# ivanalberico/End-To-End-Self-Supervised-SLAM

Hardware: AMD Instinct MI355X
Metric: online refinement steps/sec @640x480, seq_len=60 (higher is better)
Workload: dtype f32

## Files before the change

### end-to-end-self-supervised-slam_amd/e2ehip/_lib.py

```python
import ctypes
import os

import torch

_HERE = os.path.dirname(os.path.abspath(__file__))
LIB_PATH = os.path.join(os.path.dirname(_HERE), "lib", "libe2eslam_hip.so")

c_fp = ctypes.c_void_p
c_int = ctypes.c_int
c_i64 = ctypes.c_int64
c_f32 = ctypes.c_float


class Strides(ctypes.Structure):
    _fields_ = [("sb", c_i64), ("sc", c_i64), ("sh", c_i64), ("sw", c_i64)]


class WgradReduceDesc(ctypes.Structure):
    _fields_ = [("slabs", c_fp), ("dw", c_fp), ("dbias", c_fp), ("scale", c_fp)] + \
               [(n, c_int) for n in ("S", "Mpad", "Npad", "Cout", "Cin", "KH", "KW", "has_bias", "accumulate", "zl")] + [("first_item", ctypes.c_longlong)]


class CopyDesc(ctypes.Structure):
    _fields_ = [("src", c_fp), ("dst", c_fp), ("bytes", ctypes.c_longlong), ("first_item", ctypes.c_longlong)]


class E2EError(RuntimeError):
    pass


SIGNATURES = {
    "e2e_version": [],
    "e2e_last_error": [],
    "e2e_backproject_fwd": [c_fp, c_fp, c_fp, c_int, c_int, c_int, c_fp],
    "e2e_backproject_bwd": [c_fp, c_fp, c_fp, c_int, c_int, c_int, c_fp],
    "e2e_project3d_fwd": [c_fp, c_fp, c_fp, c_fp, c_fp, c_fp, c_int, c_int, c_int, c_fp],
    "e2e_project3d_bwd": [c_fp, c_fp, c_fp, c_fp, c_fp, c_fp, c_int, c_int, c_int, c_fp],
    "e2e_grid_sample_fwd": [c_fp, Strides, c_fp, c_fp] + [c_int] * 8 + [c_fp],
    "e2e_grid_sample_bwd": [c_fp, Strides, c_fp, c_fp, c_fp, c_fp] + [c_int] * 8 + [c_fp],
    "e2e_grid_sample_bwd_exact": [c_fp, Strides, c_fp, c_fp, c_fp, c_fp, c_fp] + [c_int] * 8 + [c_fp],
    "e2e_photometric_fwd": [c_fp, Strides, c_fp, Strides, c_fp, c_fp, c_int, c_int, c_int, c_int, c_fp],
    "e2e_photometric_bwd": [c_fp, Strides, c_fp, Strides, c_fp, c_fp, c_fp, c_int, c_int, c_int, c_int, c_fp],
    "e2e_warp_photo_workspace_floats": [c_int, c_int, c_int],
    "e2e_warp_photo_fwd": [c_fp, c_fp, Strides, c_fp, Strides, c_fp, c_fp, c_fp, c_fp, c_fp, c_fp, c_int, c_int, c_int,
                           c_fp, c_fp, c_fp, c_fp, c_fp, c_int, c_int, c_int, c_fp],
    "e2e_warp_photo_bwd": [c_fp, c_fp, Strides, c_fp, Strides, c_fp, c_fp, c_fp, c_fp, c_fp, c_int, c_int, c_int,
                           c_fp, c_fp, c_fp, c_fp, c_fp, c_fp, c_int, c_int, c_int, c_fp],
# ... 83 lines not shown
    "e2e_conv2d_bwd_pair_deferred": [c_fp, c_fp, c_int, c_fp] + [c_int] * 13 + [c_fp, c_int, c_fp, c_fp, c_fp, c_fp, c_fp, c_int, c_int, c_fp, c_fp, c_fp,
                                     c_int, c_f32, c_f32, ctypes.POINTER(WgradReduceDesc), c_int, c_fp],
    "e2e_wgrad_reduce_batch_prepare": [ctypes.POINTER(WgradReduceDesc), c_int],
    "e2e_wgrad_reduce_batched": [c_fp, c_int, ctypes.c_longlong, c_fp],
    "e2e_copy_batch_prepare": [ctypes.POINTER(CopyDesc), c_int],
    "e2e_copy_batched": [c_fp, c_int, ctypes.c_longlong, c_fp],
    "e2e_head_bwd_act": [c_fp, c_fp, c_fp, c_fp, c_fp, c_fp, c_fp, c_int, c_int, c_int, c_int, c_int, c_fp],
    "e2e_conv2d_act_bwd_acc": [c_fp, c_fp, c_fp, c_fp, c_i64, c_int, c_int, c_int, c_fp],
    "e2e_conv2d_gather_adjoint": [c_fp] + [c_int] * 7 + [c_fp, c_fp, c_int, c_int, c_fp],
    "e2e_conv2d_wgrad_workspace_floats": [c_int] * 8,
    "e2e_conv2d_bwd_weight": [c_fp, c_fp, c_fp, c_int, c_int, c_fp, c_fp, c_fp] + [c_int] * 13 + [c_f32, c_f32, c_fp],
    "e2e_maxpool3x3s2_fwd": [c_fp, c_fp, c_int, c_int, c_int, c_int, c_fp],
    "e2e_maxpool3x3s2_bwd": [c_fp, c_fp, c_fp, c_int, c_int, c_int, c_int, c_int, c_int, c_fp],
    "e2e_maxpool3x3s2_fwd_idx": [c_fp, c_fp, c_fp, c_int, c_int, c_int, c_int, c_fp],
    "e2e_maxpool3x3s2_bwd_idx": [c_fp, c_fp, c_fp, c_fp, c_int, c_int, c_int, c_int, c_int, c_int, c_fp],
    "e2e_bn_fold": [c_fp, c_fp, c_fp, c_fp, c_f32, c_fp, c_fp, c_fp, c_int, c_fp],
    "e2e_affine_fwd": [c_fp, c_fp, c_fp, c_fp, c_int, c_fp, c_i64, c_int, c_fp],
    "e2e_affine_bwd_workspace_floats": [c_int],
    "e2e_affine_bwd": [c_fp, c_fp, c_fp, c_fp, c_i64, c_int, c_fp, c_fp, c_int, c_fp, c_fp],
    "e2e_upsample2_concat": [c_fp, c_fp, c_fp, c_int, c_int, c_int, c_int, c_int, c_fp],
    "e2e_head_fwd": [c_fp, c_fp, c_fp, c_fp, c_int, c_int, c_int, c_int, c_int, c_fp],
    "e2e_head_workspace_floats": [],
    "e2e_head_bwd": [c_fp, c_fp, c_fp, c_fp, c_fp, c_fp, c_fp, c_int, c_int, c_int, c_int, c_fp],
    "e2e_icp_workspace_bytes": [],
    "e2e_icp_state_doubles": [],
    "e2e_icp_state_init": [c_fp, c_fp, c_fp, c_fp, c_fp, ctypes.c_double, c_fp],
    "e2e_icp_update": [c_fp, c_fp, c_fp, c_fp, c_fp, c_fp, c_int, c_int, ctypes.c_double, ctypes.c_double, ctypes.c_double, ctypes.c_double, c_fp],
    "e2e_icp_reduce_update": [c_fp, c_fp, c_fp, c_fp, c_fp, c_f32, c_i64, c_fp, c_fp, c_fp, c_fp, c_fp, c_fp, c_int, c_int,
                              ctypes.c_double, ctypes.c_double, ctypes.c_double, ctypes.c_double, c_fp],
    "e2e_icp_source_subsample": [c_fp, c_fp, c_int, c_int, c_int, c_fp, c_fp, c_fp],
    "e2e_pf_active_subsample_dev": [c_fp, c_fp, c_fp, c_i64, c_fp, c_int, c_int, c_int, c_fp, c_fp, c_fp, c_i64, c_fp],
    "e2e_icp_normal_equations": [c_fp, c_fp, c_fp, c_fp, c_fp, c_f32, c_i64, c_fp, c_fp, c_fp],
}
_RESTYPE = {"e2e_last_error": ctypes.c_char_p, "e2e_warp_photo_workspace_floats": c_i64,
            "e2e_warp_photo_lossgrad_workspace_floats": c_i64, "e2e_pf_workspace_bytes": c_i64,
            "e2e_warp_photo_terms_lossgrad_workspace_floats": c_i64, "e2e_smoothness_norm_lossgrad_workspace_floats": c_i64,
            "e2e_knn1_workspace_bytes": c_i64, "e2e_knn1_index_capacity_bytes": c_i64, "e2e_knn1_index_capacity_bytes_res": c_i64, "e2e_median_workspace_bytes": c_i64,
            "e2e_depth_scale_workspace_bytes": c_i64, "e2e_reduce_workspace_floats": c_i64,
            "e2e_conv2d_wgrad_workspace_floats": c_i64, "e2e_conv2d_wgrad_tuned_workspace_floats": c_i64, "e2e_conv_tuned_workspace_floats": c_i64, "e2e_conv2d_splitk_workspace_floats": c_i64, "e2e_conv2d_bwd_data_workspace_floats": c_i64,
            "e2e_head_workspace_floats": c_i64, "e2e_icp_workspace_bytes": c_i64, "e2e_icp_state_doubles": c_i64, "e2e_aux_workspace_floats": c_i64,
            "e2e_affine_bwd_workspace_floats": c_i64, "e2e_wgrad_reduce_batch_prepare": ctypes.c_longlong, "e2e_copy_batch_prepare": ctypes.c_longlong}

_lib = None


def load():
    global _lib
    if _lib is None:
        if not os.path.exists(LIB_PATH):
            raise E2EError(f"{LIB_PATH} not found: build it with `python __graft_entry__.py build` "
                           "(there is no CPU / PyTorch fallback for the hot path)")
        lib = ctypes.CDLL(LIB_PATH)
        for name, args in SIGNATURES.items():
            fn = getattr(lib, name)
            fn.argtypes = args
            fn.restype = _RESTYPE.get(name, c_int)
        _lib = lib
    return _lib


PROFILE_HOOK = [None]


def call(name, *args):
    lib = load()
    hook = PROFILE_HOOK[0]
    rc = getattr(lib, name)(*args) if hook is None else hook.around(name, args, lambda: getattr(lib, name)(*args))
    if rc != 0:
        raise E2EError(f"{name} failed ({rc}): {lib.e2e_last_error().decode()}")


def stream():
    return torch.cuda.current_stream().cuda_stream


def dev(t, name="tensor", dtype=torch.float32):
    if not torch.is_tensor(t):
        raise TypeError(f"{name}: expected a torch.Tensor, got {type(t).__name__}")
    if not t.is_cuda:
        raise E2EError(f"{name}: the e2eslam hot path runs on the HIP device only (got a {t.device} tensor); "
                       "there is no CPU fallback")
    if t.dtype != dtype:
        raise TypeError(f"{name}: expected {dtype}, got {t.dtype}")
    return t


def ptr(t):
    return None if t is None else ctypes.c_void_p(t.data_ptr())


def strides4(t):
    s = t.stride()
    return Strides(s[0], s[1], s[2], s[3])
```

### end-to-end-self-supervised-slam_amd/e2ehip/netplan.py

```python
import ctypes
import os

import torch

from . import _lib as L
from .conv import ACT, _ld, epoch_sum

_f32 = torch.float32
PAIR_WGRAD_FIRST = 0


class Buf:
    __slots__ = ("t", "g", "written", "B", "h", "w", "C", "act")

    def __init__(self, B, h, w, C, dev, need_grad=True, act=0):
        self.B, self.h, self.w, self.C = B, h, w, C
        self.act = act
        self.t = torch.empty(B, h, w, C, device=dev, dtype=_f32)
        self.g = torch.empty(B, h, w, C, device=dev, dtype=_f32) if need_grad else None
        self.written = False

    def nchw(self):
        return self.t.permute(0, 3, 1, 2)

# ... 101 lines not shown
        s, s1 = self, self.src1
        L.call("e2e_conv2d_gather_adjoint_act", L.ptr(s.dxp), s.src0.B, s.Hs, s.Ws, s.Cin, s.C1, s.up, 1 if s.pp else 0, L.ptr(s.src0.g),
               L.ptr(s1.g) if s1 is not None else None, 1 if s.src0.written else 0, 1 if (s1 is not None and s1.written) else 0,
               L.ptr(s.src0.t), s.src0.act, L.ptr(s1.t) if s1 is not None else None, s1.act if s1 is not None else 0, st)
        s.src0.written = True
        if s1 is not None:
            s1.written = True


class _Head:

    def __init__(self, plan, src, weight, bias, act):
        self.src, self.weight, self.bias, self.act = src, weight, bias, ACT[act]
        self.out = Buf(src.B, src.h, src.w, 1, plan.dev)
        self.dz = torch.empty_like(self.out.t)
        self.ws = torch.empty(L.load().e2e_head_workspace_floats(), device=plan.dev, dtype=_f32)

    def fwd(self, plan, st, slot=None):
        s = self.src
        L.call("e2e_head_fwd", _at(s.t, slot), L.ptr(self.weight), L.ptr(self.bias), _at(self.out.t, slot), s.B if slot is None else 1, s.h, s.w, s.C, self.act, st)

    def bwd(self, plan, st):
        s, n = self.src, self.out.t.numel()
        L.call("e2e_conv2d_act_bwd", L.ptr(self.out.g), L.ptr(self.out.t), None, L.ptr(self.dz), n, 1, self.act, st)
        if s.written:
            raise RuntimeError("the disparity head's input has a single consumer")
        L.call("e2e_head_bwd_act", L.ptr(self.dz), L.ptr(s.t), L.ptr(self.weight), L.ptr(s.g), L.ptr(plan.sink(self.weight)),
               L.ptr(plan.sink(self.bias)) if self.bias is not None else None, L.ptr(self.ws), s.B, s.h, s.w, s.C, s.act, st)
        s.written = True


class _MaxPool:
    def __init__(self, plan, src):
        self.src = src
        self.out = Buf(src.B, (src.h - 1) // 2 + 1, (src.w - 1) // 2 + 1, src.C, plan.dev)
        self.argmax = torch.empty(self.out.t.shape, device=plan.dev, dtype=torch.uint8)

    def fwd(self, plan, st, slot=None):
        s = self.src
        L.call("e2e_maxpool3x3s2_fwd_idx", _at(s.t, slot), _at(self.out.t, slot), _at(self.argmax, slot), s.B if slot is None else 1, s.h, s.w, s.C, st)

    def bwd(self, plan, st):
        s = self.src
        if s.act not in (0, ACT["relu"]):
            raise NotImplementedError("launch plan: the max-pool follows a ReLU (ResNet stem)")
        L.call("e2e_maxpool3x3s2_bwd_idx", L.ptr(s.t), L.ptr(self.argmax), L.ptr(self.out.g), L.ptr(s.g), s.B, s.h, s.w, s.C, 1 if s.written else 0,
               1 if s.act else 0, st)
        s.written = True


class _BNAffine:

    def __init__(self, plan, src, bn_mod):
        self.src, self.bn = src, bn_mod
        C = src.C
        self.out = Buf(src.B, src.h, src.w, C, plan.dev)
        self.scale, self.shift, self.rstd = (torch.empty(C, device=plan.dev, dtype=_f32) for _ in range(3))
        self.ws = torch.empty(L.load().e2e_affine_bwd_workspace_floats(C), device=plan.dev, dtype=_f32)

    def fwd(self, plan, st, slot=None):
        b, s = self.bn, self.src
        L.call("e2e_bn_fold", L.ptr(b.weight), L.ptr(b.bias), L.ptr(b.running_mean), L.ptr(b.running_var), float(b.eps), L.ptr(self.scale),
               L.ptr(self.shift), L.ptr(self.rstd), s.C, st)
        L.call("e2e_affine_fwd", _at(s.t, slot), L.ptr(self.scale), L.ptr(self.shift), None, 0, _at(self.out.t, slot),
               s.t.numel() if slot is None else s.t[0].numel(), s.C, st)

    def bwd(self, plan, st):
        b, s = self.bn, self.src
        n = s.t.numel()
        L.call("e2e_affine_bwd", L.ptr(self.out.g), L.ptr(s.t), L.ptr(b.running_mean), L.ptr(self.rstd), n // s.C, s.C, L.ptr(plan.sink(b.weight)),
               L.ptr(plan.sink(b.bias)), 0, L.ptr(self.ws), st)
        if s.act != 0:
            raise NotImplementedError("launch plan: a trainable BatchNorm follows a plain convolution")
        L.call("e2e_conv2d_act_bwd_acc", L.ptr(self.out.g), L.ptr(self.out.g), L.ptr(self.scale), L.ptr(s.g), n, s.C, 0, 1 if s.written else 0, st)
        s.written = True


class NetPlan:
    def __init__(self, model, B, H, W, device, overlap=True):
        from depth_estimation.networks import BasicBlock
        self.model, self.dev, self.overlap = model, torch.device(device), overlap
        self.paired = os.environ.get("E2E_PAIRED_BWD", "1") != "0"
        self.B, self.H, self.W = B, H, W
        if H % 32 or W % 32:
            raise ValueError(f"launch plan: the encoder halves the image five times and the decoder doubles it back before every skip "
                             f"concatenation (networks.py:277-292): height and width must be multiples of 32, got {H} x {W}")
        self.ops, self._sinks, self._side = [], {}, None
        enc, dec = model.encoder.encoder, model.decoder
        if any(m.training for m in model.modules() if isinstance(m, torch.nn.BatchNorm2d)):
            raise NotImplementedError("the launch plan runs BatchNorm in eval mode (refinement mode, online_adaption.py:175-184)")
        self.x = Buf(B, H, W, 3, self.dev, need_grad=False)

        def bn_args(bn):
            return (bn.weight, bn.bias, bn.running_mean, bn.running_var, bn.eps)

        def conv_bn(src, conv, bn, relu, residual=None, in_norm=None):
            if bn.weight.requires_grad or bn.bias.requires_grad:
                if relu or residual is not None or in_norm is not None:
                    raise NotImplementedError("launch plan: a trainable BatchNorm is expected on the downsample branches only (set_refinement_mode)")
                z = self._add(_Conv(self, src, None, conv.weight, None, None, None, None, conv.stride[0], conv.padding[0], "zeros", 1, None))
                return self._add(_BNAffine(self, z, bn))
            return self._add(_Conv(self, src, None, conv.weight, None, bn_args(bn), residual, "relu" if relu else None, conv.stride[0],
                                   conv.padding[0], "zeros", 1, in_norm))

        f = conv_bn(self.x, enc.conv1, enc.bn1, True, in_norm=(0.45, 1.0 / 0.225))
# ... 16 lines not shown
                        c2.res_via, c1.pre_from = c1, c2
                elif isinstance(idt_op, _BNAffine) and idt.act == 0:
                    idt.g = c2.out.g
                    c2.res_aliased = True
            feats.append(x)
        self.features = feats
        x = feats[-1]
        for i in range(4, -1, -1):
            c0, c1 = dec.convs[("upconv", i, 0)].conv, dec.convs[("upconv", i, 1)].conv
            x = self._add(_Conv(self, x, None, c0.conv.weight, c0.conv.bias, None, None, "elu", 1, 1, c0.pad_mode, 1, None))
            skip = feats[i - 1] if (dec.use_skips and i > 0) else None
            x = self._add(_Conv(self, x, skip, c1.conv.weight, c1.conv.bias, None, None, "elu", 1, 1, c1.pad_mode, 2, None))
        hc = dec.convs[("dispconv", 0)]
        if tuple(hc.conv.weight.shape) != (1, 16, 3, 3) or hc.pad_mode != "reflect":
            raise NotImplementedError("launch plan: the indoor decoder's 16 -> 1 reflect head")
        self.head = _Head(self, x, hc.conv.weight, hc.conv.bias, "disp")
        self.ops.append(self.head)
        self.disp = self.head.out
        self._desc = None
        self._desc_key = None
        self._retired_tables = []
        self._move_tables = {}
        self._reduce_tables = {}

    def _add(self, op):
        self.ops.append(op)
        return op.out

    def parameters(self):
        out = []
        for op in self.ops:
            if isinstance(op, _Conv) or isinstance(op, _Head):
                out.append(op.weight)
                if op.bias is not None:
                    out.append(op.bias)
            elif isinstance(op, _BNAffine):
                out += [op.bn.weight, op.bn.bias]
        return out

    def sink(self, p):
        s = self._sinks.get(id(p))
        if s is None or s.data_ptr() != _sink_of(p).data_ptr():
            s = self._sinks[id(p)] = _sink_of(p)
            if not s.is_contiguous() or tuple(s.shape) != tuple(p.shape):
                raise RuntimeError("gradient sink of a parameter must be a contiguous tensor of the parameter's shape")
        return s

    def refresh_layouts(self, st=None):
        convs = [op for op in self.ops if isinstance(op, _Conv)]
        key = tuple(op.weight.data_ptr() for op in convs)
        if self._desc is None or self._desc_key != key:
            self._desc = torch.tensor([op.layout_row() for op in convs], dtype=torch.int64).to(self.dev)
            self._desc_key = key
        L.call("e2e_conv_weight_layouts_batched", L.ptr(self._desc), len(convs), st if st is not None else L.stream())
        self.mark_layouts_current()

    def _stamp(self):
        ws = [op.weight for op in self.ops if isinstance(op, _Conv)]
        return (tuple(w.data_ptr() for w in ws), tuple(w._version for w in ws), epoch_sum(ws))

    def mark_layouts_current(self):
        self._epoch = self._stamp()

    def layouts_current(self):
        return self._desc is not None and getattr(self, "_epoch", None) == self._stamp()

    def fork(self, st):
        if not self.overlap:
            return st
        if self._side is None:
            self._side = torch.cuda.Stream(self.dev)
            self._record_side_stream_use()
        self._side.wait_stream(torch.cuda.current_stream(self.dev))
        self._forked = True
        return ctypes.c_void_p(self._side.cuda_stream)

    def join(self):
        if self.overlap and self._side is not None and getattr(self, "_forked", False):
            torch.cuda.current_stream(self.dev).wait_stream(self._side)
            self._forked = False

    def _record_side_stream_use(self):
        seen = set()
        for op in self.ops:
            ts = [op.out.t, op.out.g]
            if isinstance(op, _Conv):
                ts += [op.scale, op.ws_w, op.src0.t, op.src1.t if op.src1 is not None else None]
                for p in (op.weight, op.bias):
                    if p is not None:
                        ts.append(_sink_of(p))
            for t in ts:
                if t is not None and t.is_cuda and t.untyped_storage().data_ptr() not in seen:
                    seen.add(t.untyped_storage().data_ptr())
                    t.record_stream(self._side)

    def close(self):
        if self._side is not None:
            self._side.synchronize()
        torch.cuda.current_stream(self.dev).synchronize()
        self.ops, self._sinks, self._desc, self._reduce_tables = [], {}, None, {}

    def forward(self, frames=None):
        if frames is not None:
            self.x.t.copy_(frames)
        st = L.stream()
        for op in self.ops:
            op.fwd(self, st)
        return self.disp.t.view(self.B, 1, self.H, self.W)

    def forward_one(self, slot):
        if not 0 <= slot < self.B:
            raise ValueError("slot out of range")
        st = L.stream()
        for op in self.ops:
            op.fwd(self, st, slot)

    def move_slot(self, src, dst):
        held = self._move_tables.get((src, dst))
        if held is None:
            if not 0 <= src < self.B or not 0 <= dst < self.B or src == dst:
                raise ValueError("slots out of range")
            if torch.cuda.is_current_stream_capturing():
                raise RuntimeError("launch plan: move_slot builds its copy table on first use; run it eagerly once before capturing it")
            pairs = []
            for op in self.ops:
                pairs.append((op.out.t[src], op.out.t[dst]))
                if isinstance(op, _MaxPool):
                    pairs.append((op.argmax[src], op.argmax[dst]))
            if any(a.numel() * a.element_size() % 16 or a.data_ptr() % 16 or b.data_ptr() % 16 for a, b in pairs):
                for a, b in pairs:
                    b.copy_(a)
                return
            arr = (L.CopyDesc * len(pairs))(*[L.CopyDesc(a.data_ptr(), b.data_ptr(), a.numel() * a.element_size(), 0) for a, b in pairs])
            total = L.load().e2e_copy_batch_prepare(arr, len(pairs))
            if total <= 0:
# ... 70 lines not shown
```

### end-to-end-self-supervised-slam_amd/e2ehip/optim.py

```python
import torch

from . import _lib as L


class FlatParams:

    def __init__(self, params):
        params = [p for p in params]
        if not params:
            raise ValueError("no parameters")
        dev = params[0].device
        offs, total = [], 0
        for p in params:
            offs.append(total)
            total += (p.numel() + 3) // 4 * 4
        self.params, self.offsets, self.numel = params, offs, total
        self.data = torch.zeros(total, device=dev, dtype=torch.float32)
        self.grad_ext = torch.zeros(total + 4, device=dev, dtype=torch.float32)
        self.grad = self.grad_ext[:total]
        self.grad_ext[total] = 1.0
        with torch.no_grad():
            for p, o in zip(params, offs):
                self.data[o:o + p.numel()].copy_(p.reshape(-1))
                p.data = self.data[o:o + p.numel()].view_as(p)
# ... 18 lines not shown

    def zero_grad(self):
        self.grad.zero_()
        self.bind_grads()

    def participants(self):
        return self.grad_ext[self.numel:self.numel + 1]


class FusedAdam(torch.optim.Optimizer):

    SCHEDULE_LEN = 1 << 18

    def __init__(self, params, lr=1e-3, betas=(0.9, 0.999), eps=1e-8):
        params = list(params)
        super().__init__(params, dict(lr=lr, betas=betas, eps=eps, weight_decay=0, amsgrad=False))
        if len(self.param_groups) != 1:
            raise NotImplementedError("FusedAdam steps ONE parameter group (one lr / betas / eps for the flat bucket)")
        self._all = list(self.param_groups[0]["params"])
        self._pending = None
        self.flat = None
        self.steps = 0
        self._sched = self._sched_key = self._counter = None

    def _resident_state(self):
        g = self.param_groups[0]
        key = (float(g["lr"]), float(g["betas"][0]), float(g["betas"][1]))
        dev = self.flat.data.device
        if self._counter is None:
            self._counter = torch.ones(1, device=dev, dtype=torch.int32)
            self._sched = torch.empty(self.SCHEDULE_LEN, 2, device=dev, dtype=torch.float32)
        if self._sched_key != key:
            t = torch.arange(1, self.SCHEDULE_LEN + 1, dtype=torch.float64)
            bc1 = 1.0 - torch.pow(torch.tensor(key[1], dtype=torch.float64), t)
            bc2 = 1.0 - torch.pow(torch.tensor(key[2], dtype=torch.float64), t)
            self._sched.copy_(torch.stack([key[0] / bc1, torch.sqrt(bc2)], 1).to(torch.float32))
            self._sched_key = key
        return self._sched, self._counter

    def steps_done(self):
        return 0 if self._counter is None else int(self._counter.item()) - 1

    def _build(self):
        act = [p for p in self._all if p.requires_grad and p.grad is not None]
        if not act:
            raise RuntimeError("FusedAdam.step(): no parameter has a gradient")
        grads = [p.grad.detach().clone() for p in act]
        self.flat = FlatParams(act)
        with torch.no_grad():
            for p, g in zip(act, grads):
                p.grad.copy_(g)
        self.m = torch.zeros_like(self.flat.data)
        self.v = torch.zeros_like(self.flat.data)
# ... 73 lines not shown
            for i, st in state.items():
                if i in offs:
                    o, n = offs[i]
                    self.m[o:o + n].copy_(st["exp_avg"].reshape(-1))
                    self.v[o:o + n].copy_(st["exp_avg_sq"].reshape(-1))
        self._resident_state()
        self._counter.fill_(t + 1)

    def zero_grad(self, set_to_none=True):
        if self.flat is None:
            for p in self._all:
                p.grad = None
        else:
            self.flat.zero_grad()

    @torch.no_grad()
    def step(self, closure=None):
        if self.flat is None:
            self._build()
        g = self.param_groups[0]
        self.steps += 1
        self.flat.touched()
        sched, counter = self._resident_state()
        L.call("e2e_adam_step_resident", L.ptr(self.flat.data), L.ptr(self.flat.grad), L.ptr(self.flat.participants()), L.ptr(self.m), L.ptr(self.v),
               self.flat.numel, float(g["betas"][0]), float(g["betas"][1]), float(g["eps"]), L.ptr(sched), self.SCHEDULE_LEN, L.ptr(counter), L.stream())
```

### end-to-end-self-supervised-slam_amd/e2ehip/stepplan.py

```python
import torch

from . import _lib as L
from . import dist as edist
from .fused import LossGradPlan, TermsLossGradPlan
from .netplan import NetPlan
from .ops import fusion_alpha_den

_f32 = torch.float32


class RefineStepPlan:
    def __init__(self, model, optimizer, H, W, device, padding_mode="border", use_mask=True, reg_kind="l2", w_reg=1e-2, w_3d=1.0, sigma=0.6,
                 overlap=True, use_graphs=True, geometric=False, smoothness=False, auto_masking=False, min_reprojection=False,
                 w_geometric=0.5, w_smoothness=1e-3):
        self.dev, self.H, self.W, self.N = torch.device(device), H, W, H * W
        self.opt, self.use_graphs, self.w_3d = optimizer, use_graphs, float(w_3d)
        self.net = NetPlan(model, 2, H, W, self.dev, overlap=overlap)
        optimizer.prebuild(model.used_parameters())
        if {id(p) for p in self.net.parameters()} != {id(p) for p in model.used_parameters() if p.requires_grad}:
            raise RuntimeError("launch plan and model disagree about the trainable parameters")
        f = dict(device=self.dev, dtype=_f32)
        lib = L.load()
        self.colors = self.net.x.t
        self.gt = torch.zeros(2, H, W, 1, **f)
# ... 32 lines not shown
        self.map_pose_src, self.map_pose_tgt = (torch.eye(4, **f).reshape(1, 4, 4).clone() for _ in range(2))
        self._pstream = None
        self.median_elements_override = None
        self.net.refresh_layouts()

    def set_pair(self, colors_prev, colors_cur, gt_prev, gt_cur, K, T_host, pose_tgt, inv_K=None, pose_src=None):
        self.colors[0].copy_(colors_prev)
        self.colors[1].copy_(colors_cur)
        self.gt[0].copy_(gt_prev)
        self.gt[1].copy_(gt_cur)
        self.K[0].copy_(K)
        self.inv_K[0].copy_(torch.pinverse(K) if inv_K is None else inv_K)
        self.T[0].copy_(T_host, non_blocking=True)
        self.pose_tgt[0].copy_(pose_tgt)
        if pose_src is not None:
            self.pose_src[0].copy_(pose_src)
        L.call("e2e_median_lower", L.ptr(self.gt), self.gt.numel(), L.ptr(self.median_gt), L.ptr(self.ws_med), L.stream())

    def _run(self, key, fn):
        if getattr(self, "_closed", False):
            raise RuntimeError("RefineStepPlan used after close()")
        if not self.use_graphs or L.PROFILE_HOOK[0] is not None:
            return fn()
        g = self._graphs.get(key)
        if g is not None:
            return g.replay()
        fn()
        cur = torch.cuda.current_stream(self.dev)
        if self._gstream is None:
            self._gstream = torch.cuda.Stream(self.dev)
        self._gstream.wait_stream(cur)
        g = torch.cuda.CUDAGraph()
        with torch.cuda.stream(self._gstream):
            with torch.cuda.graph(g, stream=self._gstream, capture_error_mode="thread_local"):
                fn()
        cur.wait_stream(self._gstream)
        self._graphs[key] = g

    def _forward(self):
        st = L.stream()
        disp = self.net.forward()
        L.call("e2e_depth_scale_fwd", L.ptr(disp), L.ptr(self.median_gt), L.ptr(self.delta), L.ptr(self.depth), L.ptr(self.md), L.ptr(self.ratio),
               L.ptr(self.ws_scale), disp.numel(), st)

    def stash_map_inputs(self):
        self.map_rgb.copy_(self.colors)
# ... 158 lines not shown
```

### include/e2eslam.h

```cpp
#ifndef E2ESLAM_H
#define E2ESLAM_H

#include <stdint.h>

#ifdef __cplusplus
extern "C" {
#endif

#define E2E_OK 0
#define E2E_ERR_ARG (-1)
#define E2E_ERR_LAUNCH (-2)
#define E2E_ERR_WORKSPACE (-3)

#define E2E_PADDING_ZEROS 0
#define E2E_PADDING_BORDER 1

typedef struct e2e_strides {
    int64_t sb, sc, sh, sw;
} e2e_strides;

int e2e_version(void);
const char* e2e_last_error(void);


// ... 303 lines not shown
                             int accumulate, int mul_relu, void* stream);

int e2e_bn_fold(const float* gamma, const float* beta, const float* running_mean,
                const float* running_var, float eps, float* scale, float* shift, float* rstd, int C,
                void* stream);
int e2e_affine_fwd(const float* z, const float* scale, const float* shift, const float* residual, int relu,
                   float* y, int64_t n, int C, void* stream);
int64_t e2e_affine_bwd_workspace_floats(int C);
int e2e_affine_bwd(const float* dy, const float* z, const float* mean, const float* rstd, int64_t P,
                   int C, float* dgamma, float* dbeta, int accumulate, float* workspace, void* stream);

int e2e_upsample2_concat(const float* x, const float* skip, float* y, int B, int h, int w, int C1,
                         int C2, void* stream);

int e2e_head_fwd(const float* x, const float* w, const float* bias, float* y, int B, int H, int W,
                 int Cin, int act, void* stream);
int64_t e2e_head_workspace_floats(void);
int e2e_head_bwd(const float* dz, const float* x, const float* w, float* dx, float* dw, float* dbias,
                 float* workspace, int B, int H, int W, int Cin, void* stream);

int e2e_head_bwd_act(const float* dz, const float* x, const float* w, float* dx, float* dw, float* dbias,
                     float* workspace, int B, int H, int W, int Cin, int in_act, void* stream);


int64_t e2e_icp_workspace_bytes(void);
int e2e_icp_normal_equations(const float* src, const float* tgt, const float* tgt_normals,
                             const long long* idx, const float* dists, float dist_thresh, int64_t n,
                             double* out29, void* workspace, void* stream);

int64_t e2e_icp_state_doubles(void);
int e2e_icp_state_init(double* state, float* T32, float* step32, const float* prev_pose, float* pose_out,
                       double damp, void* stream);
int e2e_icp_update(const double* out29, double* state, float* T32, float* step32, const float* prev_pose,
                   float* pose_out, int mode, int phase, double lambda_max, double B, double B2, double nu,
                   void* stream);
int e2e_icp_reduce_update(const float* src, const float* tgt, const float* tgt_normals, const long long* idx,
                          const float* dists, float dist_thresh, int64_t n, void* workspace, double* state, float* T32,
                          float* step32, const float* prev_pose, float* pose_out, int mode, int phase,
                          double lambda_max, double B, double B2, double nu, void* stream);
int e2e_icp_source_subsample(const float* Vg, const float* depth, int H, int W, int dsratio, float* src,
                             int* status, void* stream);

int64_t e2e_aux_workspace_floats(void);

int e2e_smoothness_lossgrad(const float* disp, const float* img, e2e_strides img_strides, int B, int C,
                            int H, int W, float* loss_out, float* g_disp, float* workspace,
// ... 31 lines not shown
```

Baseline: 214.0.

## Fuse step tail kernels: batched BN fold, fused affine/head backward, single-pass Adam

Adds a new HIP translation unit that fuses several tail-of-step operations. BatchNorm folds become one batched launch driven by a device descriptor table, and that table is refreshed only when the BN tensors change. The affine backward now also writes dz and finishes its cross-slice reduction with a last-workgroup ticket. The head backward applies the output activation derivative inline, and Adam increments its step counter in-kernel via a ticket. The aim is fewer kernel launches and memory passes per refinement step, at the cost of atomics and ticket state plus extra host-side version checks on BN tensors.

```diff
diff --git a/end-to-end-self-supervised-slam_amd/csrc/step_tail.hip b/end-to-end-self-supervised-slam_amd/csrc/step_tail.hip
--- /dev/null
+++ b/end-to-end-self-supervised-slam_amd/csrc/step_tail.hip
@@ -0,0 +1,311 @@
+#include "e2e_common.h"
+
+#include <math.h>
+
+typedef float f4v __attribute__((ext_vector_type(4)));
+
+enum { ACT_NONE = 0, ACT_RELU = 1, ACT_ELU = 2, ACT_DISP = 3 };
+
+#define HC 16
+#define HEAD_PARTS 2048
+#define AFF_SLICES 64
+#define DT 256
+
+__device__ __forceinline__ float load_published(const float* p) {
+    return __int_as_float(__hip_atomic_load((const int*)p, __ATOMIC_RELAXED, __HIP_MEMORY_SCOPE_AGENT));
+}
+
+__device__ __forceinline__ bool last_workgroup(int* ticket, int expected) {
+    __shared__ int s_last;
+    __threadfence();
+    __syncthreads();
+    if (threadIdx.x == 0) s_last = (__hip_atomic_fetch_add(ticket, 1, __ATOMIC_ACQ_REL, __HIP_MEMORY_SCOPE_AGENT) == expected - 1) ? 1 : 0;
+    __syncthreads();
+    const bool last = s_last != 0;
+    if (last) __threadfence();
+    return last;
+}
+
+__device__ __forceinline__ float act_bwd_value(float g, float v, int act) {
+    if (act == ACT_RELU) g = v > 0.f ? g : 0.f;
+    else if (act == ACT_ELU) g = v > 0.f ? g : g * (v + 1.f);
+    else if (act == ACT_DISP) { const float s = (v - 0.01f) * 0.1f; g = g * 10.f * s * (1.f - s); }
+    return g;
+}
+
+__device__ __forceinline__ float act_deriv(float y, int act) {
+    if (act == ACT_RELU) return y > 0.f ? 1.f : 0.f;
+    if (act == ACT_ELU) return y > 0.f ? 1.f : y + 1.f;
+    return 1.f;
+}
+
+__global__ __launch_bounds__(256) void k_bn_fold_batched(const e2e_bn_fold_desc* __restrict__ d) {
+    const e2e_bn_fold_desc e = d[blockIdx.y];
+    const int c = blockIdx.x * 256 + threadIdx.x;
+    if (c >= e.C) return;
+    const float r = 1.f / sqrtf(e.running_var[c] + e.eps);
+    const float s = e.gamma[c] * r;
+    e.scale[c] = s;
+    e.shift[c] = e.beta[c] - e.running_mean[c] * s;
+    if (e.rstd) e.rstd[c] = r;
+}
+
+__global__ __launch_bounds__(256) void k_affine_bwd_fused(const float* __restrict__ dy, const float* __restrict__ z, const float* __restrict__ mean,
+                                                          const float* __restrict__ rstd, const float* __restrict__ scale, int64_t P, int C,
+                                                          int64_t pix_per_slice, float* __restrict__ partial , int* __restrict__ tickets,
+                                                          float* __restrict__ dgamma, float* __restrict__ dbeta, int accumulate, float* __restrict__ dz,
+                                                          int dz_accumulate) {
+    __shared__ float sg[4][64], sb[4][64];
+    const int cl = threadIdx.x & 63, pl = threadIdx.x >> 6;
+    const int c = blockIdx.x * 64 + cl;
+    const int64_t p0 = (int64_t)blockIdx.y * pix_per_slice, p1 = (p0 + pix_per_slice < P) ? p0 + pix_per_slice : P;
+    float ag = 0.f, ab = 0.f;
+    if (c < C) {
+        const float m = mean ? mean[c] : 0.f, r = rstd ? rstd[c] : 1.f;
+        for (int64_t p = p0 + pl; p < p1; p += 4) {
+            const float g = dy[p * C + c];
+            ag = fmaf(g, (z[p * C + c] - m) * r, ag);
+            ab += g;
+            if (dz) {
+                float gs = g;
+                if (scale) gs *= scale[c];
+                dz[p * C + c] = dz_accumulate ? dz[p * C + c] + gs : gs;
+            }
+        }
+    }
+    sg[pl][cl] = ag;
+    sb[pl][cl] = ab;
+    __syncthreads();
+    if (pl == 0 && c < C) {
+        float* o = partial + (int64_t)blockIdx.y * 2 * C;
+        o[c] = ((sg[0][cl] + sg[1][cl]) + sg[2][cl]) + sg[3][cl];
+        o[C + c] = ((sb[0][cl] + sb[1][cl]) + sb[2][cl]) + sb[3][cl];
+    }
+    const int S = (int)gridDim.y;
+    if (!last_workgroup(tickets + blockIdx.x, S)) return;
+    const int w = pl;
+    float g = 0.f, b = 0.f;
+    if (c < C)
+        for (int s = w; s < S; s += 4) {
+            g += load_published(partial + (int64_t)s * 2 * C + c);
+            b += load_published(partial + (int64_t)s * 2 * C + C + c);
+        }
+    sg[w][cl] = g;
+    sb[w][cl] = b;
+    __syncthreads();
+    if (w == 0 && c < C) {
+        g = ((sg[0][cl] + sg[1][cl]) + sg[2][cl]) + sg[3][cl];
+        b = ((sb[0][cl] + sb[1][cl]) + sb[2][cl]) + sb[3][cl];
+        if (dgamma) dgamma[c] = accumulate ? dgamma[c] + g : g;
+        if (dbeta) dbeta[c] = accumulate ? dbeta[c] + b : b;
+    }
+    if (threadIdx.x == 0) tickets[blockIdx.x] = 0;
+}
+
+__global__ __launch_bounds__(256) void k_head_bwd_data_act(const float* __restrict__ gy, const float* __restrict__ y, int out_act,
+                                                           const float* __restrict__ w, float* __restrict__ dx, int B, int H, int W,
+                                                           const float* __restrict__ xin, int dact) {
+    __shared__ float sw[9 * HC];
+    for (int i = threadIdx.x; i < 9 * HC; i += 256) {
+        const int ci = i / 9, tap = i - ci * 9;
+        sw[tap * HC + ci] = w[i];
+    }
+    __syncthreads();
+    const int64_t N = (int64_t)B * H * W;
+    const int cq = threadIdx.x & 3;
+    for (int64_t n = (int64_t)blockIdx.x * 64 + (threadIdx.x >> 2); n < N; n += (int64_t)gridDim.x * 64) {
+        const int b = (int)(n / ((int64_t)H * W));
+        const int r = (int)(n - (int64_t)b * H * W), h = r / W, ww = r - h * W;
+        f4v acc = {0.f, 0.f, 0.f, 0.f};
+        const int ry = (h == 1) ? 0 : ((h == H - 2) ? H + 1 : -100);
+        const int rx = (ww == 1) ? 0 : ((ww == W - 2) ? W + 1 : -100);
+        const float* gz = gy + (int64_t)b * H * W;
+        const float* yz = y + (int64_t)b * H * W;
+#define DZ_AT(o) act_bwd_value(gz[o], yz[o], out_act)
+#pragma unroll
+        for (int kh = 0; kh < 3; ++kh)
+#pragma unroll
+            for (int kw = 0; kw < 3; ++kw) {
+                const float* wt = &sw[(kh * 3 + kw) * HC + cq * 4];
+                const int qy0 = h - kh + 1, qx0 = ww - kw + 1, qy1 = ry - kh, qx1 = rx - kw;
+                const bool y0 = qy0 >= 0 && qy0 < H, x0 = qx0 >= 0 && qx0 < W, y1 = qy1 >= 0 && qy1 < H, x1 = qx1 >= 0 && qx1 < W;
+                float g = (y0 && x0) ? DZ_AT((int64_t)qy0 * W + qx0) : 0.f;
+                if (y1 | x1) {
+                    if (y0 && x1) g += DZ_AT((int64_t)qy0 * W + qx1);
+                    if (y1 && x0) g += DZ_AT((int64_t)qy1 * W + qx0);
+                    if (y1 && x1) g += DZ_AT((int64_t)qy1 * W + qx1);
+                }
+#pragma unroll
+                for (int c = 0; c < 4; ++c) acc[c] = fmaf(g, wt[c], acc[c]);
+            }
+#undef DZ_AT
+        if (dact) {
+            const f4v xv = *(const f4v*)(xin + n * HC + cq * 4);
+#pragma unroll
+            for (int e = 0; e < 4; ++e) acc[e] *= act_deriv(xv[e], dact);
+        }
+        *(f4v*)(dx + n * HC + cq * 4) = acc;
+    }
+}
+
+__global__ __launch_bounds__(256) void k_head_bwd_weight_act(const float* __restrict__ gy, const float* __restrict__ y, int out_act,
+                                                             const float* __restrict__ x, float* __restrict__ partials, int B, int H, int W) {
+    __shared__ float red[4][9 * HC + 1];
+    const int64_t N = (int64_t)B * H * W;
+    const int lane = threadIdx.x & 63, wave = threadIdx.x >> 6, cq = threadIdx.x & 3, ps = threadIdx.x >> 2;
+    const int64_t per = (N + gridDim.x - 1) / gridDim.x;
+    const int64_t n0 = (int64_t)blockIdx.x * per, n1 = (n0 + per < N) ? n0 + per : N;
+    float acc[36];
+#pragma unroll
+    for (int k = 0; k < 36; ++k) acc[k] = 0.f;
+    float sb = 0.f;
+    for (int64_t n = n0 + ps; n < n1; n += 64) {
+        const float g = act_bwd_value(gy[n], y[n], out_act);
+        const int b = (int)(n / ((int64_t)H * W));
+        const int r = (int)(n - (int64_t)b * H * W), h = r / W, ww = r - h * W;
+#pragma unroll
+        for (int kh = 0; kh < 3; ++kh)
+#pragma unroll
+            for (int kw = 0; kw < 3; ++kw) {
+                const int ys = reflect1(h + kh - 1, H), xs = reflect1(ww + kw - 1, W);
+                const f4v v = *(const f4v*)(x + (((int64_t)b * H + ys) * W + xs) * HC + cq * 4);
+#pragma unroll
+                for (int c = 0; c < 4; ++c) acc[(kh * 3 + kw) * 4 + c] = fmaf(g, v[c], acc[(kh * 3 + kw) * 4 + c]);
+            }
+        sb += g;
+    }
+#pragma unroll
+    for (int k = 0; k < 36; ++k) {
+        float v = acc[k];
+#pragma unroll
+        for (int o = 4; o < 64; o <<= 1) v += __shfl_xor(v, o, 64);
+        acc[k] = v;
+    }
+#pragma unroll
+    for (int o = 4; o < 64; o <<= 1) sb += __shfl_xor(sb, o, 64);
+    if (lane < 4) {
+#pragma unroll
+        for (int t = 0; t < 9; ++t)
+#pragma unroll
+            for (int c = 0; c < 4; ++c) red[wave][t * HC + lane * 4 + c] = acc[t * 4 + c];
+        if (lane == 0) red[wave][9 * HC] = sb;
+    }
+    __syncthreads();
+    if (threadIdx.x < 9 * HC + 1)
+        partials[(int64_t)blockIdx.x * (9 * HC + 1) + threadIdx.x] = ((red[0][threadIdx.x] + red[1][threadIdx.x]) + red[2][threadIdx.x]) + red[3][threadIdx.x];
+}
+
+__global__ __launch_bounds__(256) void k_head_wreduce_tail(const float* __restrict__ partials, int nparts, float* __restrict__ dw, float* __restrict__ dbias) {
+    __shared__ float red[4];
+    const int col = blockIdx.x;
+    float s = 0.f;
+    for (int i = threadIdx.x; i < nparts; i += 256) s += partials[(int64_t)i * (9 * HC + 1) + col];
+    const float t = block_sum(s, red);
+    if (threadIdx.x == 0) {
+        if (col == 9 * HC) { if (dbias) dbias[0] = t; }
+        else { const int tap = col / HC, ci = col - tap * HC; dw[ci * 9 + tap] = t; }
+    }
+}
+
+__global__ __launch_bounds__(DT) void k_adam_advancing(float* __restrict__ p, const float* __restrict__ g, float* __restrict__ m, float* __restrict__ v,
+                                                       int64_t n, float one_minus_b1, float b2, float one_minus_b2, float eps,
+                                                       const float* __restrict__ participants, const float2* __restrict__ schedule,
+                                                       int* __restrict__ step_counter, int schedule_len, int* __restrict__ ticket) {
+    const int64_t n4 = n >> 2;
+    const float cnt = participants ? fmaxf(participants[0], 1.f) : 1.f;
+    const int t0 = __hip_atomic_load(step_counter, __ATOMIC_RELAXED, __HIP_MEMORY_SCOPE_AGENT);
+    const int t = t0 < 1 ? 1 : (t0 > schedule_len ? schedule_len : t0);
+    const float2 sc = schedule[t - 1];
+    const float step_size = sc.x, bc2_sqrt = sc.y;
+    float4* p4 = (float4*)p; const float4* g4 = (const float4*)g; float4* m4 = (float4*)m; float4* v4 = (float4*)v;
+    for (int64_t i = (int64_t)blockIdx.x * DT + threadIdx.x; i < n4; i += (int64_t)gridDim.x * DT) {
+        float4 pp = p4[i], gg = g4[i], mm = m4[i], vv = v4[i];
+        float* pa = (float*)&pp; float* ga = (float*)&gg; float* ma = (float*)&mm; float* va = (float*)&vv;
+#pragma unroll
+        for (int k = 0; k < 4; ++k) {
+            ga[k] = ga[k] / cnt;
+            ma[k] = ma[k] + one_minus_b1 * (ga[k] - ma[k]);
+            va[k] = va[k] * b2 + one_minus_b2 * (ga[k] * ga[k]);
+            const float den = sqrtf(va[k]) / bc2_sqrt + eps;
+            pa[k] = pa[k] - step_size * (ma[k] / den);
+        }
+        p4[i] = pp; m4[i] = mm; v4[i] = vv;
+    }
+    for (int64_t i = (n4 << 2) + (int64_t)blockIdx.x * DT + threadIdx.x; i < n; i += (int64_t)gridDim.x * DT) {
+        const float gi = g[i] / cnt;
+        const float mi = m[i] + one_minus_b1 * (gi - m[i]);
+        const float vi = v[i] * b2 + one_minus_b2 * (gi * gi);
+        m[i] = mi; v[i] = vi;
+        p[i] = p[i] - step_size * (mi / (sqrtf(vi) / bc2_sqrt + eps));
+    }
+    if (!last_workgroup(ticket, (int)gridDim.x)) return;
+    if (threadIdx.x == 0) {
+        step_counter[0] = t0 + 1;
+        ticket[0] = 0;
+    }
+}
+
+static inline int egrid(int64_t n) { int64_t g = (n + 255) / 256; return (int)(g < 1 ? 1 : (g > 4096 ? 4096 : g)); }
+static inline int sgrid(int64_t n, int cap) {
+    int64_t g = (n + DT - 1) / DT;
+    return (int)(g < 1 ? 1 : (g > cap ? cap : g));
+}
+
+extern "C" {
+
+int e2e_bn_fold_batched(const e2e_bn_fold_desc* descs_dev, int n, int max_channels, void* stream) {
+    E2E_REQUIRE(descs_dev && n > 0 && max_channels > 0, E2E_ERR_ARG, "e2e_bn_fold_batched: bad argument");
+    hipLaunchKernelGGL(k_bn_fold_batched, dim3((max_channels + 255) / 256, n), dim3(256), 0, (hipStream_t)stream, descs_dev);
+    E2E_LAUNCH_CHECK("e2e_bn_fold_batched");
+    return E2E_OK;
+}
+
+int64_t e2e_affine_bwd_fused_workspace_floats(int C) {
+    const int64_t c = C > 0 ? C : 1;
+    return (int64_t)AFF_SLICES * 2 * c + (c + 63) / 64;
+}
+
+int e2e_affine_bwd_fused(const float* dy, const float* z, const float* mean, const float* rstd, const float* scale, int64_t P, int C,
+                         float* dgamma, float* dbeta, int accumulate, float* dz, int dz_accumulate, float* workspace, void* stream) {
+    E2E_REQUIRE(dy && z && workspace && P > 0 && C > 1 && (dgamma || dbeta) && dz != dy && dz != z, E2E_ERR_ARG,
+                "e2e_affine_bwd_fused: bad argument (C > 1; dz must not alias dy or z)");
+    int S = AFF_SLICES;
+    int64_t pps = (P + S - 1) / S;
+    if (pps < 4) pps = 4;
+    S = (int)((P + pps - 1) / pps);
+    int* tickets = (int*)(workspace + (int64_t)AFF_SLICES * 2 * C);
+    hipLaunchKernelGGL(k_affine_bwd_fused, dim3((C + 63) / 64, S), dim3(256), 0, (hipStream_t)stream, dy, z, mean, rstd, scale, P, C, pps, workspace,
+                       tickets, dgamma, dbeta, accumulate, dz, dz_accumulate);
+    E2E_LAUNCH_CHECK("e2e_affine_bwd_fused");
+    return E2E_OK;
+}
+
+int e2e_head_bwd_fused(const float* g, const float* y, int out_act, const float* x, const float* w, float* dx, float* dw, float* dbias,
+                       float* workspace, int B, int H, int W, int Cin, int in_act, void* stream) {
+    E2E_REQUIRE(g && y && x && w && workspace && B > 0 && H >= 2 && W >= 2 && Cin == HC && in_act >= 0 && in_act <= 2 && out_act >= 0 && out_act <= 3,
+                E2E_ERR_ARG, "e2e_head_bwd_fused: bad argument");
+    E2E_REQUIRE((int64_t)B * H * W * HC < (1ll << 31), E2E_ERR_ARG, "e2e_head_bwd_fused: activation too large for 32-bit element offsets");
+    hipStream_t st = (hipStream_t)stream;
+    if (dx) hipLaunchKernelGGL(k_head_bwd_data_act, dim3(egrid((int64_t)B * H * W * 4)), dim3(256), 0, st, g, y, out_act, w, dx, B, H, W, x, in_act);
+    if (dw) {
+        hipLaunchKernelGGL(k_head_bwd_weight_act, dim3(HEAD_PARTS), dim3(256), 0, st, g, y, out_act, x, workspace, B, H, W);
+        hipLaunchKernelGGL(k_head_wreduce_tail, dim3(9 * HC + 1), dim3(256), 0, st, workspace, HEAD_PARTS, dw, dbias);
+    }
+    E2E_LAUNCH_CHECK("e2e_head_bwd_fused");
+    return E2E_OK;
+}
+
+int e2e_adam_step_resident_fused(float* params, const float* grad_sums, const float* participants, float* exp_avg, float* exp_avg_sq, int64_t n,
+                                 float beta1, float beta2, float eps, const float* schedule, int schedule_len, int* step_counter, int* ticket,
+                                 void* stream) {
+    E2E_REQUIRE(n > 0 && params && grad_sums && exp_avg && exp_avg_sq && schedule && schedule_len > 0 && step_counter && ticket, E2E_ERR_ARG,
+                "e2e_adam_step_resident_fused: bad argument");
+    E2E_REQUIRE(((uintptr_t)params | (uintptr_t)grad_sums | (uintptr_t)exp_avg | (uintptr_t)exp_avg_sq) % 16 == 0 && (uintptr_t)schedule % 8 == 0,
+                E2E_ERR_ARG, "e2e_adam_step_resident_fused: buffers must be 16-byte aligned");
+    hipLaunchKernelGGL(k_adam_advancing, dim3(sgrid(n >> 2 > 0 ? n >> 2 : 1, 2048)), dim3(DT), 0, (hipStream_t)stream, params, grad_sums, exp_avg,
+                       exp_avg_sq, n, 1.0f - beta1, beta2, 1.0f - beta2, eps, participants, (const float2*)schedule, step_counter, schedule_len, ticket);
+    E2E_LAUNCH_CHECK("e2e_adam_step_resident_fused");
+    return E2E_OK;
+}
+
+}
diff --git a/end-to-end-self-supervised-slam_amd/e2ehip/_lib.py b/end-to-end-self-supervised-slam_amd/e2ehip/_lib.py
--- a/end-to-end-self-supervised-slam_amd/e2ehip/_lib.py
+++ b/end-to-end-self-supervised-slam_amd/e2ehip/_lib.py
@@ -23,6 +23,10 @@
 
 class CopyDesc(ctypes.Structure):
     _fields_ = [("src", c_fp), ("dst", c_fp), ("bytes", ctypes.c_longlong), ("first_item", ctypes.c_longlong)]
+
+
+class BnFoldDesc(ctypes.Structure):
+    _fields_ = [(n, c_fp) for n in ("gamma", "beta", "running_mean", "running_var", "scale", "shift", "rstd")] + [("eps", c_f32), ("C", c_int)]
 
 
 class E2EError(RuntimeError):
@@ -152,6 +156,11 @@
     "e2e_head_fwd": [c_fp, c_fp, c_fp, c_fp, c_int, c_int, c_int, c_int, c_int, c_fp],
     "e2e_head_workspace_floats": [],
     "e2e_head_bwd": [c_fp, c_fp, c_fp, c_fp, c_fp, c_fp, c_fp, c_int, c_int, c_int, c_int, c_fp],
+    "e2e_bn_fold_batched": [c_fp, c_int, c_int, c_fp],
+    "e2e_affine_bwd_fused_workspace_floats": [c_int],
+    "e2e_affine_bwd_fused": [c_fp, c_fp, c_fp, c_fp, c_fp, c_i64, c_int, c_fp, c_fp, c_int, c_fp, c_int, c_fp, c_fp],
+    "e2e_head_bwd_fused": [c_fp, c_fp, c_int, c_fp, c_fp, c_fp, c_fp, c_fp, c_fp, c_int, c_int, c_int, c_int, c_int, c_fp],
+    "e2e_adam_step_resident_fused": [c_fp, c_fp, c_fp, c_fp, c_fp, c_i64, c_f32, c_f32, c_f32, c_fp, c_int, c_fp, c_fp, c_fp],
     "e2e_icp_workspace_bytes": [],
     "e2e_icp_state_doubles": [],
     "e2e_icp_state_init": [c_fp, c_fp, c_fp, c_fp, c_fp, ctypes.c_double, c_fp],
@@ -169,7 +178,7 @@
             "e2e_depth_scale_workspace_bytes": c_i64, "e2e_reduce_workspace_floats": c_i64,
             "e2e_conv2d_wgrad_workspace_floats": c_i64, "e2e_conv2d_wgrad_tuned_workspace_floats": c_i64, "e2e_conv_tuned_workspace_floats": c_i64, "e2e_conv2d_splitk_workspace_floats": c_i64, "e2e_conv2d_bwd_data_workspace_floats": c_i64,
             "e2e_head_workspace_floats": c_i64, "e2e_icp_workspace_bytes": c_i64, "e2e_icp_state_doubles": c_i64, "e2e_aux_workspace_floats": c_i64,
-            "e2e_affine_bwd_workspace_floats": c_i64, "e2e_wgrad_reduce_batch_prepare": ctypes.c_longlong, "e2e_copy_batch_prepare": ctypes.c_longlong}
+            "e2e_affine_bwd_workspace_floats": c_i64, "e2e_affine_bwd_fused_workspace_floats": c_i64, "e2e_wgrad_reduce_batch_prepare": ctypes.c_longlong, "e2e_copy_batch_prepare": ctypes.c_longlong}
 
 _lib = None
 
@@ -200,6 +209,10 @@
         raise E2EError(f"{name} failed ({rc}): {lib.e2e_last_error().decode()}")
 
 
+def fused_tail():
+    return os.environ.get("E2E_FUSED_TAIL", "1") != "0"
+
+
 def stream():
     return torch.cuda.current_stream().cuda_stream
 
diff --git a/end-to-end-self-supervised-slam_amd/e2ehip/netplan.py b/end-to-end-self-supervised-slam_amd/e2ehip/netplan.py
--- a/end-to-end-self-supervised-slam_amd/e2ehip/netplan.py
+++ b/end-to-end-self-supervised-slam_amd/e2ehip/netplan.py
@@ -147,9 +147,15 @@
 
     def bwd(self, plan, st):
         s, n = self.src, self.out.t.numel()
-        L.call("e2e_conv2d_act_bwd", L.ptr(self.out.g), L.ptr(self.out.t), None, L.ptr(self.dz), n, 1, self.act, st)
         if s.written:
             raise RuntimeError("the disparity head's input has a single consumer")
+        if plan.fused:
+            L.call("e2e_head_bwd_fused", L.ptr(self.out.g), L.ptr(self.out.t), self.act, L.ptr(s.t), L.ptr(self.weight), L.ptr(s.g),
+                   L.ptr(plan.sink(self.weight)), L.ptr(plan.sink(self.bias)) if self.bias is not None else None, L.ptr(self.ws), s.B, s.h, s.w, s.C,
+                   s.act, st)
+            s.written = True
+            return
+        L.call("e2e_conv2d_act_bwd", L.ptr(self.out.g), L.ptr(self.out.t), None, L.ptr(self.dz), n, 1, self.act, st)
         L.call("e2e_head_bwd_act", L.ptr(self.dz), L.ptr(s.t), L.ptr(self.weight), L.ptr(s.g), L.ptr(plan.sink(self.weight)),
                L.ptr(plan.sink(self.bias)) if self.bias is not None else None, L.ptr(self.ws), s.B, s.h, s.w, s.C, s.act, st)
         s.written = True
@@ -182,21 +188,33 @@
         self.out = Buf(src.B, src.h, src.w, C, plan.dev)
         self.scale, self.shift, self.rstd = (torch.empty(C, device=plan.dev, dtype=_f32) for _ in range(3))
         self.ws = torch.empty(L.load().e2e_affine_bwd_workspace_floats(C), device=plan.dev, dtype=_f32)
+        self.ws_fused = torch.zeros(L.load().e2e_affine_bwd_fused_workspace_floats(C), device=plan.dev, dtype=_f32) if plan.fused else None
+
+    def fold_row(self):
+        b = self.bn
+        return L.BnFoldDesc(b.weight.data_ptr(), b.bias.data_ptr(), b.running_mean.data_ptr(), b.running_var.data_ptr(), self.scale.data_ptr(),
+                            self.shift.data_ptr(), self.rstd.data_ptr(), float(b.eps), self.src.C)
 
     def fwd(self, plan, st, slot=None):
         b, s = self.bn, self.src
-        L.call("e2e_bn_fold", L.ptr(b.weight), L.ptr(b.bias), L.ptr(b.running_mean), L.ptr(b.running_var), float(b.eps), L.ptr(self.scale),
-               L.ptr(self.shift), L.ptr(self.rstd), s.C, st)
+        if not plan.fused:
+            L.call("e2e_bn_fold", L.ptr(b.weight), L.ptr(b.bias), L.ptr(b.running_mean), L.ptr(b.running_var), float(b.eps), L.ptr(self.scale),
+                   L.ptr(self.shift), L.ptr(self.rstd), s.C, st)
         L.call("e2e_affine_fwd", _at(s.t, slot), L.ptr(self.scale), L.ptr(self.shift), None, 0, _at(self.out.t, slot),
                s.t.numel() if slot is None else s.t[0].numel(), s.C, st)
 
     def bwd(self, plan, st):
         b, s = self.bn, self.src
         n = s.t.numel()
+        if s.act != 0:
+            raise NotImplementedError("launch plan: a trainable BatchNorm follows a plain convolution")
+        if plan.fused:
+            L.call("e2e_affine_bwd_fused", L.ptr(self.out.g), L.ptr(s.t), L.ptr(b.running_mean), L.ptr(self.rstd), L.ptr(self.scale), n // s.C, s.C,
+                   L.ptr(plan.sink(b.weight)), L.ptr(plan.sink(b.bias)), 0, L.ptr(s.g), 1 if s.written else 0, L.ptr(self.ws_fused), st)
+            s.written = True
+            return
         L.call("e2e_affine_bwd", L.ptr(self.out.g), L.ptr(s.t), L.ptr(b.running_mean), L.ptr(self.rstd), n // s.C, s.C, L.ptr(plan.sink(b.weight)),
                L.ptr(plan.sink(b.bias)), 0, L.ptr(self.ws), st)
-        if s.act != 0:
-            raise NotImplementedError("launch plan: a trainable BatchNorm follows a plain convolution")
         L.call("e2e_conv2d_act_bwd_acc", L.ptr(self.out.g), L.ptr(self.out.g), L.ptr(self.scale), L.ptr(s.g), n, s.C, 0, 1 if s.written else 0, st)
         s.written = True
 
@@ -206,6 +224,7 @@
         from depth_estimation.networks import BasicBlock
         self.model, self.dev, self.overlap = model, torch.device(device), overlap
         self.paired = os.environ.get("E2E_PAIRED_BWD", "1") != "0"
+        self.fused = L.fused_tail()
         self.B, self.H, self.W = B, H, W
         if H % 32 or W % 32:
             raise ValueError(f"launch plan: the encoder halves the image five times and the decoder doubles it back before every skip "
@@ -268,6 +287,7 @@
         self._retired_tables = []
         self._move_tables = {}
         self._reduce_tables = {}
+        self._bn_table = self._bn_table_key = self._bn_epoch = None
 
     def _add(self, op):
         self.ops.append(op)
@@ -299,7 +319,36 @@
             self._desc = torch.tensor([op.layout_row() for op in convs], dtype=torch.int64).to(self.dev)
             self._desc_key = key
         L.call("e2e_conv_weight_layouts_batched", L.ptr(self._desc), len(convs), st if st is not None else L.stream())
+        if self.fused:
+            self.fold_bn(st)
         self.mark_layouts_current()
+
+    def _bn_tensors(self):
+        return [t for op in self.ops if isinstance(op, _BNAffine) for t in (op.bn.weight, op.bn.bias, op.bn.running_mean, op.bn.running_var)]
+
+    def _bn_stamp(self):
+        ts = self._bn_tensors()
+        return (tuple(t.data_ptr() for t in ts), tuple(t._version for t in ts), epoch_sum(ts))
+
+    def fold_bn(self, st=None):
+        bns = [op for op in self.ops if isinstance(op, _BNAffine)]
+        if not bns:
+            return
+        key = tuple(t.data_ptr() for t in self._bn_tensors())
+        if self._bn_table is None or self._bn_table_key != key:
+            if torch.cuda.is_current_stream_capturing():
+                raise RuntimeError("launch plan: the BatchNorm fold table changed under stream capture; run the plan eagerly once first")
+            if self._bn_table is not None:
+                self._retired_tables.append(self._bn_table)
+            arr = (L.BnFoldDesc * len(bns))(*[op.fold_row() for op in bns])
+            self._bn_table = torch.frombuffer(bytearray(bytes(arr)), dtype=torch.uint8).to(self.dev)
+            self._bn_table_key = key
+        L.call("e2e_bn_fold_batched", L.ptr(self._bn_table), len(bns), max(op.src.C for op in bns), st if st is not None else L.stream())
+        self._bn_epoch = self._bn_stamp()
+
+    def ensure_bn_current(self):
+        if self.fused and self._bn_epoch != self._bn_stamp():
+            self.fold_bn()
 
     def _stamp(self):
         ws = [op.weight for op in self.ops if isinstance(op, _Conv)]
@@ -307,6 +356,8 @@
 
     def mark_layouts_current(self):
         self._epoch = self._stamp()
+        if self.fused and self._bn_table is not None:
+            self._bn_epoch = self._bn_stamp()
 
     def layouts_current(self):
         return self._desc is not None and getattr(self, "_epoch", None) == self._stamp()
@@ -344,11 +395,12 @@
         if self._side is not None:
             self._side.synchronize()
         torch.cuda.current_stream(self.dev).synchronize()
-        self.ops, self._sinks, self._desc, self._reduce_tables = [], {}, None, {}
+        self.ops, self._sinks, self._desc, self._reduce_tables, self._bn_table = [], {}, None, {}, None
 
     def forward(self, frames=None):
         if frames is not None:
             self.x.t.copy_(frames)
+        self.ensure_bn_current()
         st = L.stream()
         for op in self.ops:
             op.fwd(self, st)
@@ -357,6 +409,7 @@
     def forward_one(self, slot):
         if not 0 <= slot < self.B:
             raise ValueError("slot out of range")
+        self.ensure_bn_current()
         st = L.stream()
         for op in self.ops:
             op.fwd(self, st, slot)
diff --git a/end-to-end-self-supervised-slam_amd/e2ehip/optim.py b/end-to-end-self-supervised-slam_amd/e2ehip/optim.py
--- a/end-to-end-self-supervised-slam_amd/e2ehip/optim.py
+++ b/end-to-end-self-supervised-slam_amd/e2ehip/optim.py
@@ -64,6 +64,8 @@
         self.flat = None
         self.steps = 0
         self._sched = self._sched_key = self._counter = None
+        self._fused = L.fused_tail()
+        self._ticket = None
 
     def _resident_state(self):
         g = self.param_groups[0]
@@ -71,6 +73,7 @@
         dev = self.flat.data.device
         if self._counter is None:
             self._counter = torch.ones(1, device=dev, dtype=torch.int32)
+            self._ticket = torch.zeros(1, device=dev, dtype=torch.int32)
             self._sched = torch.empty(self.SCHEDULE_LEN, 2, device=dev, dtype=torch.float32)
         if self._sched_key != key:
             t = torch.arange(1, self.SCHEDULE_LEN + 1, dtype=torch.float64)
@@ -190,5 +193,10 @@
         self.steps += 1
         self.flat.touched()
         sched, counter = self._resident_state()
+        if self._fused:
+            L.call("e2e_adam_step_resident_fused", L.ptr(self.flat.data), L.ptr(self.flat.grad), L.ptr(self.flat.participants()), L.ptr(self.m),
+                   L.ptr(self.v), self.flat.numel, float(g["betas"][0]), float(g["betas"][1]), float(g["eps"]), L.ptr(sched), self.SCHEDULE_LEN,
+                   L.ptr(counter), L.ptr(self._ticket), L.stream())
+            return
         L.call("e2e_adam_step_resident", L.ptr(self.flat.data), L.ptr(self.flat.grad), L.ptr(self.flat.participants()), L.ptr(self.m), L.ptr(self.v),
                self.flat.numel, float(g["betas"][0]), float(g["betas"][1]), float(g["eps"]), L.ptr(sched), self.SCHEDULE_LEN, L.ptr(counter), L.stream())
diff --git a/end-to-end-self-supervised-slam_amd/e2ehip/stepplan.py b/end-to-end-self-supervised-slam_amd/e2ehip/stepplan.py
--- a/end-to-end-self-supervised-slam_amd/e2ehip/stepplan.py
+++ b/end-to-end-self-supervised-slam_amd/e2ehip/stepplan.py
@@ -78,6 +78,7 @@
             raise RuntimeError("RefineStepPlan used after close()")
         if not self.use_graphs or L.PROFILE_HOOK[0] is not None:
             return fn()
+        self.net.ensure_bn_current()
         g = self._graphs.get(key)
         if g is not None:
             return g.replay()
diff --git a/include/e2eslam.h b/include/e2eslam.h
--- a/include/e2eslam.h
+++ b/include/e2eslam.h
@@ -349,6 +349,33 @@
 int e2e_head_bwd_act(const float* dz, const float* x, const float* w, float* dx, float* dw, float* dbias,
                      float* workspace, int B, int H, int W, int Cin, int in_act, void* stream);
 
+typedef struct e2e_bn_fold_desc {
+    const float* gamma;
+    const float* beta;
+    const float* running_mean;
+    const float* running_var;
+    float* scale;
+    float* shift;
+    float* rstd;
+    float eps;
+    int C;
+} e2e_bn_fold_desc;
+int e2e_bn_fold_batched(const e2e_bn_fold_desc* descs_dev, int n, int max_channels, void* stream);
+
+int64_t e2e_affine_bwd_fused_workspace_floats(int C);
+int e2e_affine_bwd_fused(const float* dy, const float* z, const float* mean, const float* rstd, const float* scale,
+                         int64_t P, int C, float* dgamma, float* dbeta, int accumulate, float* dz,
+                         int dz_accumulate, float* workspace, void* stream);
+
+int e2e_head_bwd_fused(const float* g, const float* y, int out_act, const float* x, const float* w, float* dx,
+                       float* dw, float* dbias, float* workspace, int B, int H, int W, int Cin, int in_act,
+                       void* stream);
+
+int e2e_adam_step_resident_fused(float* params, const float* grad_sums, const float* participants, float* exp_avg,
+                                 float* exp_avg_sq, int64_t n, float beta1, float beta2, float eps,
+                                 const float* schedule, int schedule_len, int* step_counter, int* ticket,
+                                 void* stream);
+
 
 int64_t e2e_icp_workspace_bytes(void);
 int e2e_icp_normal_equations(const float* src, const float* tgt, const float* tgt_normals,
```

New measurement: 191.0. -10.8%, worse.
